# AndrewRLawrence/dp_gp_lvm

Hardware: AMD Instinct MI355X
Metric: ELBO evals/sec (N=2000,D=512,M=128,Q=10) (higher is better)
Workload: dtype f32 (psi-statistics: f16 hi/lo-split MFMA operands, fp32 accumulate) + f64 (Cholesky chain)

## Files before the change

### dp_gp_lvm_amd/csrc/psi2_pairs.hip

```cpp
#include <type_traits>
#include "internal.h"
#include "psi2_consts.h"
#include "psi2_chain_task.h"

typedef _Float16 pp_h8 __attribute__((ext_vector_type(8)));
typedef _Float16 pp_h2 __attribute__((ext_vector_type(2)));
typedef float pp_f16v __attribute__((ext_vector_type(16)));

#define PP_APAD 8
#define PP_LDS_HDR 512

#ifndef PP_G
#define PP_G(KS) ((KS) <= 4 ? 6 : ((KS) <= 6 ? 4 : 2))
#endif
#ifndef PP_WAVES
#define PP_WAVES 2
#endif
template <int KS> struct PairsCfg { static constexpr int G = PP_G(KS); };

#ifndef PP_NW8_MIN_TILES
#define PP_NW8_MIN_TILES 512
#endif
#ifndef PP_DEEP_PREFETCH
#define PP_DEEP_PREFETCH 1
#endif
#ifndef PP_SCALAR_ADD
#define PP_SCALAR_ADD 1
#endif

template <int KS, int GG, int NW>
__device__ __forceinline__ void pairs_load(pp_h8 (&bop)[GG][KS], int tb, const _Float16 *__restrict__ img, int l5, int half) {
#pragma unroll
    for (int g = 0; g < GG; ++g) {
        const pp_h8 *row = reinterpret_cast<const pp_h8 *>(img) + (size_t)(tb + NW * g) * KS * 64 + 32 * half + l5;
#pragma unroll
        for (int ks = 0; ks < KS; ++ks) bop[g][ks] = row[ks * 64];
    }
}

template <int KS, int GG, int NW>
__device__ __forceinline__ void pairs_group(int tb, pp_h8 (&bop)[GG][KS], int tb_next, const _Float16 *__restrict__ aimg,
                                            const _Float16 *__restrict__ img,
                                            const unsigned *__restrict__ pmap, const float *__restrict__ scale, int ntile,
                                            int l5, int half, float poison, float *__restrict__ out, int Mp, int chunk) {
    constexpr int SLP = 16 * KS, LDA = SLP + PP_APAD;
    static_assert(GG == 1 || (GG & 1) == 0, "ping-pong needs an even number of resident tiles");
    unsigned pm[GG];
    float sc[GG], old[GG];
#pragma unroll
    for (int g = 0; g < GG; ++g) {
        pm[g] = pmap[32 * (tb + NW * g) + l5];
        sc[g] = scale[32 * (tb + NW * g) + l5];
    }
#pragma unroll
    for (int g = 0; g < GG; ++g) {
        old[g] = 0.0f;
        if (chunk && pm[g] != 0xffffffffu && half == 0) old[g] = out[(size_t)(pm[g] >> 16) * Mp + (pm[g] & 0xffffu)];
    }
    float acc[GG][4];
#pragma unroll
    for (int g = 0; g < GG; ++g)
#pragma unroll
        for (int i = 0; i < 4; ++i) acc[g][i] = 0.0f;
    const _Float16 *arow = aimg + (size_t)l5 * LDA + 8 * half;
    auto load_a = [&](pp_h8 (&a)[KS], int nt) __attribute__((always_inline)) {
#ifdef PP_DIAG_NO_ALOAD
        if (nt > 1) return;
#endif
#pragma unroll
        for (int ks = 0; ks < KS; ++ks) a[ks] = *reinterpret_cast<const pp_h8 *>(arow + (size_t)nt * 32 * LDA + 16 * ks);
    };
    auto mma = [&](pp_f16v &c, const pp_h8 (&a)[KS], const pp_h8 (&bq)[KS]) __attribute__((always_inline)) {
#pragma unroll
        for (int v = 0; v < 16; ++v) c[v] = 0.0f;
#pragma unroll
        for (int ks = 0; ks < KS; ++ks) c = __builtin_amdgcn_mfma_f32_32x32x16_f16(a[ks], bq[ks], c, 0, 0, 0);
    };
    auto stage = [&](pp_f16v &cn, const pp_h8 (&a)[KS], const pp_h8 (&bq)[KS], float (&ac)[4], const pp_f16v &cu)
                     __attribute__((always_inline)) {
#pragma unroll
        for (int v = 0; v < 16; ++v) cn[v] = 0.0f;
#ifndef PP_MFMA_PER_STEP
#define PP_MFMA_PER_STEP 1
#endif
#pragma unroll
        for (int ks = 0; ks < KS; ks += PP_MFMA_PER_STEP) {
#ifndef PP_DIAG_NO_MFMA
#pragma unroll
            for (int k2 = ks; k2 < ks + PP_MFMA_PER_STEP && k2 < KS; ++k2)
                cn = __builtin_amdgcn_mfma_f32_32x32x16_f16(a[k2], bq[k2], cn, 0, 0, 0);
#endif
            __builtin_amdgcn_sched_barrier(0);
            const int kend = (ks + PP_MFMA_PER_STEP < KS) ? ks + PP_MFMA_PER_STEP : KS;
            const int v0 = (16 * ks) / KS, v1 = (16 * kend) / KS;
#pragma unroll
            for (int v = v0; v < v1; ++v) {
#ifdef PP_DIAG_NO_EXP
                const float e = cu[v];
#else
                const float e = __builtin_amdgcn_exp2f(cu[v]);
#endif
#if PP_SCALAR_ADD
                asm("v_add_f32 %0, %0, %1" : "+v"(ac[v & 3]) : "v"(e));
#else
                ac[v & 3] += e;
#endif
            }
            __builtin_amdgcn_sched_barrier(0);
        }
    };
    pp_f16v c0, c1;
    if constexpr (GG == 2 && PP_DEEP_PREFETCH) {
        pp_h8 a0[KS], a1[KS], a2[KS];
        load_a(a0, 0);
        load_a(a1, min(1, ntile - 1));
        mma(c0, a0, bop[0]);
#pragma unroll 1
        for (int nt = 0; nt < ntile; nt += 3) {
            load_a(a2, min(nt + 2, ntile - 1));
            stage(c1, a0, bop[1], acc[0], c0);
            stage(c0, a1, bop[0], acc[1], c1);
            if (nt + 1 >= ntile) break;
            load_a(a0, min(nt + 3, ntile - 1));
            stage(c1, a1, bop[1], acc[0], c0);
            stage(c0, a2, bop[0], acc[1], c1);
            if (nt + 2 >= ntile) break;
            load_a(a1, min(nt + 4, ntile - 1));
            stage(c1, a2, bop[1], acc[0], c0);
            stage(c0, a0, bop[0], acc[1], c1);
        }
    } else {
        pp_h8 a_0[KS], a_1[KS];
        load_a(a_0, 0);
        mma(c0, a_0, bop[0]);
        auto row = [&](const pp_h8 (&a_cur)[KS], const pp_h8 (&a_nxt)[KS]) __attribute__((always_inline)) {
            if constexpr (GG == 1) {
                stage(c1, a_nxt, bop[0], acc[0], c0);
                c0 = c1;
            } else {
#pragma unroll
                for (int g = 0; g < GG; g += 2) {
                    stage(c1, a_cur, bop[g + 1], acc[g], c0);
                    if (g + 2 < GG) stage(c0, a_cur, bop[g + 2], acc[g + 1], c1);
                    else stage(c0, a_nxt, bop[0], acc[g + 1], c1);
                }
            }
        };
#pragma unroll 1
        for (int nt = 0; nt < ntile; nt += 2) {
            load_a(a_1, min(nt + 1, ntile - 1));
            row(a_0, a_1);
            if (nt + 1 >= ntile) break;
            load_a(a_0, min(nt + 2, ntile - 1));
            row(a_1, a_0);
        }
    }
    if (tb_next >= 0) pairs_load<KS, GG, NW>(bop, tb_next, img, l5, half);
#pragma unroll
    for (int g = 0; g < GG; ++g) {
        float tot = (acc[g][0] + acc[g][1]) + (acc[g][2] + acc[g][3]);
        tot += __shfl_xor(tot, 32, 64);
        if (pm[g] != 0xffffffffu && half == 0)
            out[(size_t)(pm[g] >> 16) * Mp + (pm[g] & 0xffffu)] = old[g] + (sc[g] * tot + poison);
    }
}

template <typename TIN>
__global__ __launch_bounds__(256) void psi2_pair_scale_kernel(int M, int Q, const TIN *__restrict__ z,
                                                              const TIN *__restrict__ gamma, const TIN *__restrict__ alpha,
                                                              float *__restrict__ scale) {
    psi2_pair_scale_block<TIN, TIN>((int)blockIdx.y, (int)blockIdx.x, M, Q, z, gamma, alpha, scale);
}

template <typename TIN, int KS, int NW>
__global__ __launch_bounds__(64 * NW, PP_WAVES) void psi2_pairs_kernel(int N, int M, int Q, int B, const unsigned char *__restrict__ consts,
                                                            const TIN *__restrict__ mu, const TIN *__restrict__ s,
                                                            const TIN *__restrict__ gamma, const float *__restrict__ scale,
                                                            float *__restrict__ part, int Mp, int n_per_split, int n_splits,
                                                            int n_ranges, int tiles_per_range, int R, ChainKTask task) {
    constexpr int G = PairsCfg<KS>::G, SLP = 16 * KS, LDA = SLP + PP_APAD;
    extern __shared__ __align__(16) unsigned char smem_raw[];
    int item;
    if (psi2_task_1d(blockIdx.x, task.ws ? B : 0, task.last != 0, item)) {
#ifndef PP_NO_CHAIN
        if constexpr (std::is_same<TIN, double>::value && NW == 4) chain_k_task<2>(task, item, smem_raw);
#endif
        return;
    }
    const int b = item % B, sp = (item / B) % n_splits, rg = item / (B * n_splits);
    float *gq = reinterpret_cast<float *>(smem_raw);
    float *zc = gq + 32;
    _Float16 *aimg = reinterpret_cast<_Float16 *>(smem_raw + PP_LDS_HDR);
    const Psi2Consts C = psi2_consts_layout(M, Q);
    const _Float16 *img = reinterpret_cast<const _Float16 *>(consts + C.off_pairs);
    const unsigned *pmap = reinterpret_cast<const unsigned *>(consts + C.off_pmap);
    const float *sc_b = scale + (size_t)b * C.Ppad;
    const int t = threadIdx.x, lane = t & 63, l5 = lane & 31, half = lane >> 5;
    const int wv = __builtin_amdgcn_readfirstlane(t >> 6);
    if (t < 32) {
        gq[t] = (t < Q) ? (float)gamma[(size_t)b * Q + t] : 0.0f;
        zc[t] = reinterpret_cast<const float *>(consts)[t];
    }
    const int tiles_total = C.Ppad / 32;
    const int t0 = rg * tiles_per_range, t1 = min(tiles_total, t0 + tiles_per_range);
    const int nbeg = sp * n_per_split, nend = min(N, nbeg + n_per_split);
    float poison = 0.0f;
    float *out = part + ((size_t)sp * B + b) * (size_t)Mp * Mp;
    bool oor = false;
    __syncthreads();

    for (int n0 = nbeg, chunk = 0; n0 < nend; n0 += R, ++chunk) {
        const int rows = min(R, nend - n0), ntile = (rows + 31) >> 5;
        if (chunk) __syncthreads();
        for (int r = t; r < 32 * ntile; r += 64 * NW) {
            const int n = n0 + r;
            unsigned *dst = reinterpret_cast<unsigned *>(aimg + (size_t)r * LDA);
            float cc = -60000.0f;
            if (n < nend) {
                cc = 0.0f;
                for (int q = 0; q < Q; ++q) {
                    const float g = gq[q], sv = (float)s[(size_t)n * Q + q], mc = (float)mu[(size_t)n * Q + q] - zc[q];
                    const float den = 2.0f * g * sv + 1.0f, w = g / den;
                    const float a = dpgp_pin((float)(-0.25 * DPGP_LOG2E / PSI2_PAIR_S2_SCALE) * w);
                    const float bb = dpgp_pin((float)DPGP_LOG2E * w * mc);
                    cc -= bb * mc + 0.5f * __builtin_amdgcn_logf(den);
                    const _Float16 ah = (_Float16)a, alo = (_Float16)(a - (float)ah);
                    const _Float16 bh = (_Float16)bb, blo = (_Float16)(bb - (float)bh);
                    const pp_h2 w0 = {ah, ah}, w1 = {alo, bh}, w2 = {bh, blo};
                    dst[3 * q] = __builtin_bit_cast(unsigned, w0);
                    dst[3 * q + 1] = __builtin_bit_cast(unsigned, w1);
                    dst[3 * q + 2] = __builtin_bit_cast(unsigned, w2);
                }
                oor |= !(cc >= -8192.0f);
                cc = fmaxf(cc, -60000.0f);
            } else {
                for (int q = 0; q < 3 * Q; ++q) dst[q] = 0u;
            }
            cc = dpgp_pin(cc);
            const _Float16 ch = (_Float16)cc;
            const float r1 = dpgp_pin(cc - (float)ch);
            const _Float16 cm = (_Float16)r1;
            const pp_h2 cw = {ch, cm}, cw2 = {(_Float16)(r1 - (float)cm), (_Float16)0.0f};
            dst[3 * Q] = __builtin_bit_cast(unsigned, cw);
            for (int k = 3 * Q + 1; k < SLP / 2; ++k) dst[k] = 0u;
            if (6 * Q + 2 < SLP) dst[3 * Q + 1] = __builtin_bit_cast(unsigned, cw2);
        }
        if (__syncthreads_or(oor ? 1 : 0)) poison = __builtin_nanf("");

        int tb = t0 + wv;
        if (tb + NW * (G - 1) < t1) {
            pp_h8 bop[G][KS];
            pairs_load<KS, G, NW>(bop, tb, img, l5, half);
            for (; tb + NW * (G - 1) < t1; tb += NW * G) {
                const int nx = tb + NW * G;
                pairs_group<KS, G, NW>(tb, bop, nx + NW * (G - 1) < t1 ? nx : -1, aimg, img, pmap, sc_b, ntile, l5, half, poison, out,
                                   Mp, chunk);
            }
        }
        if constexpr (G > 2)
            for (; tb + NW < t1; tb += 2 * NW) {
                pp_h8 bop[2][KS];
                pairs_load<KS, 2, NW>(bop, tb, img, l5, half);
                pairs_group<KS, 2, NW>(tb, bop, -1, aimg, img, pmap, sc_b, ntile, l5, half, poison, out, Mp, chunk);
            }
        for (; tb < t1; tb += NW) {
            pp_h8 bop[1][KS];
            pairs_load<KS, 1, NW>(bop, tb, img, l5, half);
            pairs_group<KS, 1, NW>(tb, bop, -1, aimg, img, pmap, sc_b, ntile, l5, half, poison, out, Mp, chunk);
        }
    }
}

struct PairsGeom {
    int KS, R, n_ranges, tiles_per_range, NW;
    size_t lds;
};
static PairsGeom pairs_geom(int B, int N, int M, int Q, int ns, size_t chain_lds) {
    const Psi2Consts C = psi2_consts_layout(M, Q);
    PairsGeom g;
    g.KS = C.KS;
    const size_t row = sizeof(_Float16) * (size_t)(16 * C.KS + PP_APAD);
    size_t budget = 80 * 1024;
    if (const char *e = getenv("DPGP_PP_LDS_KB")) budget = (size_t)atoi(e) * 1024;
    if (chain_lds > budget) budget = chain_lds;
    int rmax = (int)((budget - PP_LDS_HDR) / row) & ~31;
    const int nper = dpgp_ceil_div(N, ns);
    g.NW = (!chain_lds && nper > rmax && C.Ppad / 32 >= PP_NW8_MIN_TILES) ? 8 : 4;
    if (const char *e = getenv("DPGP_PP_NW")) {
        const int v = atoi(e);
        if ((v == 4 || v == 8) && !(v == 8 && chain_lds)) g.NW = v;
    }
    if (g.NW == 8) {
        budget = 160 * 1024;
        rmax = (int)((budget - PP_LDS_HDR) / row) & ~31;
    }
    int r = dpgp_round_up(nper, 32);
    if (r > rmax) {
        const int chunks = dpgp_ceil_div(nper, rmax);
        r = dpgp_round_up(dpgp_ceil_div(nper, chunks), 32);
    }
    g.R = r;
    g.lds = PP_LDS_HDR + row * (size_t)r;
    if (chain_lds > g.lds) g.lds = chain_lds;
    const int tiles = C.Ppad / 32;
    int nr = chain_lds ? (B < 128 ? 512 - B : 512) / (B * ns) : dpgp_ceil_div(g.NW == 8 ? 256 : 512, B * ns);
    if (nr > dpgp_ceil_div(tiles, 32)) nr = dpgp_ceil_div(tiles, 32);
    if (nr < 1) nr = 1;
    if (const char *e = getenv("DPGP_PP_RANGES")) {
        const int v = atoi(e);
        if (v >= 1 && v <= tiles) nr = v;
    }
    g.tiles_per_range = dpgp_ceil_div(tiles, nr);
    g.n_ranges = dpgp_ceil_div(tiles, g.tiles_per_range);
    return g;
}

template <typename TIN, int KS, int NW>
static int launch_pairs_ks(int B, int N, int M, int Q, const TIN *mu, const TIN *s, const TIN *gamma, const float *scale,
                           float *part, int ns, const ChainKTask &task, const unsigned char *consts, const PairsGeom &g,
                           hipStream_t st) {
    const int Mp = dpgp_round_up(M, 16);
    const int nper = dpgp_ceil_div(N, ns);
    const long long nwg = (long long)B * ns * g.n_ranges + (task.ws ? B : 0);
    if (nwg > 0x7fffffffLL) return -1;
    auto kern = psi2_pairs_kernel<TIN, KS, NW>;
    if (NW == 8 && task.ws) return -16;
    if (g.lds > 48 * 1024 &&
        hipFuncSetAttribute(reinterpret_cast<const void *>(kern), hipFuncAttributeMaxDynamicSharedMemorySize, (int)g.lds) !=
            hipSuccess)
        return DPGP_ERR_LAUNCH;
    DPGP_PRELAUNCH(); hipLaunchKernelGGL(kern, dim3((unsigned)nwg), dim3(64 * NW), g.lds, st, N, M, Q, B, consts, mu, s, gamma, scale, part,
                       Mp, nper, ns, g.n_ranges, g.tiles_per_range, g.R, task);
    DPGP_LAUNCH_CHECK();
    return DPGP_OK;
}

size_t psi2_pairs_scale_bytes(int B, int M) {
    const size_t ppad = ((size_t)M * (M + 1) / 2 + 31) & ~(size_t)31;
    return dpgp_align256(sizeof(float) * (size_t)B * ppad);
}
template <typename TIN>
int launch_psi2_pairs(int B, int N, int M, int Q, const TIN *z, const TIN *mu, const TIN *s, const TIN *gamma,
                      const TIN *alpha, float *part, int ns, const ChainKTask &task, const unsigned char *consts, float *scale,
                      int scale_ready, hipStream_t st) {
    if (!consts || !scale) return -18;
    if (!scale_ready) {
        const Psi2Consts C = psi2_consts_layout(M, Q);
        DPGP_PRELAUNCH(); hipLaunchKernelGGL((psi2_pair_scale_kernel<TIN>), dim3(dpgp_ceil_div(C.Ppad, 256), B), dim3(256), 0, st, M, Q, z,
                           gamma, alpha, scale);
        DPGP_LAUNCH_CHECK();
    }
    size_t chain_lds = 0;
    if (task.ws) {
        if (!chain_k_resident(task.Mp, task.elem)) return -16;
        chain_lds = chain_k_lds_bytes(task.Mp, task.elem);
    }
    const PairsGeom g = pairs_geom(B, N, M, Q, ns, chain_lds);
    switch (g.KS) {
#define CASE(k)                                                                                                       \
    case k:                                                                                                           \
        return g.NW == 8 ? launch_pairs_ks<TIN, k, 8>(B, N, M, Q, mu, s, gamma, scale, part, ns, task, consts, g, st) \
                         : launch_pairs_ks<TIN, k, 4>(B, N, M, Q, mu, s, gamma, scale, part, ns, task, consts, g, st);
        CASE(2) CASE(4) CASE(6) CASE(8)
#undef CASE
    }
    return -4;
}
template int launch_psi2_pairs<float>(int, int, int, int, const float *, const float *, const float *, const float *,
                                      const float *, float *, int, const ChainKTask &, const unsigned char *, float *, int,
                                      hipStream_t);
template int launch_psi2_pairs<double>(int, int, int, int, const double *, const double *, const double *, const double *,
                                       const double *, float *, int, const ChainKTask &, const unsigned char *, float *, int,
                                       hipStream_t);
```

Measured before the change: 771.5.

## Peel final pipeline iteration and overlap next-group B-operand refill with tail MFMAs

Restructures the psi2 pairs MFMA pipeline so the last row is peeled out of the loop. The B-operand registers for the next tile group are refilled one slot at a time, interleaved with the tail stage and drain, instead of being loaded all at once after the loop. This is meant to hide the global-load latency of the next group behind the remaining MFMA/exp work and to avoid the redundant clamped tail iteration. It adds a REFILL template parameter and changes loop bounds, which risks edge-case bugs for small ntile values and adds register pressure.

```diff
diff --git a/dp_gp_lvm_amd/csrc/psi2_pairs.hip b/dp_gp_lvm_amd/csrc/psi2_pairs.hip
--- a/dp_gp_lvm_amd/csrc/psi2_pairs.hip
+++ b/dp_gp_lvm_amd/csrc/psi2_pairs.hip
@@ -28,6 +28,19 @@
 #define PP_SCALAR_ADD 1
 #endif
 
+__device__ __forceinline__ void pairs_accumulate(float &acc, float x) {
+#ifdef PP_DIAG_NO_EXP
+    const float e = x;
+#else
+    const float e = __builtin_amdgcn_exp2f(x);
+#endif
+#if PP_SCALAR_ADD
+    acc = dpgp_pin(acc + e);
+#else
+    acc += e;
+#endif
+}
+
 template <int KS, int GG, int NW>
 __device__ __forceinline__ void pairs_load(pp_h8 (&bop)[GG][KS], int tb, const _Float16 *__restrict__ img, int l5, int half) {
 #pragma unroll
@@ -38,7 +51,7 @@
     }
 }
 
-template <int KS, int GG, int NW>
+template <int KS, int GG, int NW, bool REFILL>
 __device__ __forceinline__ void pairs_group(int tb, pp_h8 (&bop)[GG][KS], int tb_next, const _Float16 *__restrict__ aimg,
                                             const _Float16 *__restrict__ img,
                                             const unsigned *__restrict__ pmap, const float *__restrict__ scale, int ntile,
@@ -94,20 +107,26 @@
             const int kend = (ks + PP_MFMA_PER_STEP < KS) ? ks + PP_MFMA_PER_STEP : KS;
             const int v0 = (16 * ks) / KS, v1 = (16 * kend) / KS;
 #pragma unroll
-            for (int v = v0; v < v1; ++v) {
-#ifdef PP_DIAG_NO_EXP
-                const float e = cu[v];
-#else
-                const float e = __builtin_amdgcn_exp2f(cu[v]);
-#endif
-#if PP_SCALAR_ADD
-                asm("v_add_f32 %0, %0, %1" : "+v"(ac[v & 3]) : "v"(e));
-#else
-                ac[v & 3] += e;
-#endif
-            }
+            for (int v = v0; v < v1; ++v) pairs_accumulate(ac[v & 3], cu[v]);
             __builtin_amdgcn_sched_barrier(0);
         }
+    };
+    auto drain = [&](float (&ac)[4], const pp_f16v &cu) __attribute__((always_inline)) {
+#pragma unroll
+        for (int v = 0; v < 16; ++v) pairs_accumulate(ac[v & 3], cu[v]);
+        __builtin_amdgcn_sched_barrier(0);
+    };
+    auto refill = [&](int g) __attribute__((always_inline)) {
+        if constexpr (!REFILL) return;
+        const pp_h8 *src = reinterpret_cast<const pp_h8 *>(img) + (size_t)(tb_next + NW * g) * KS * 64;
+        const unsigned lo = 32u * half + l5;
+#pragma unroll
+        for (int ks = 0; ks < KS; ++ks) bop[g][ks] = src[ks * 64 + lo];
+        __builtin_amdgcn_sched_barrier(0);
+    };
+    auto copy_a = [&](pp_h8 (&d)[KS], const pp_h8 (&a)[KS]) __attribute__((always_inline)) {
+#pragma unroll
+        for (int ks = 0; ks < KS; ++ks) d[ks] = a[ks];
     };
     pp_f16v c0, c1;
     if constexpr (GG == 2 && PP_DEEP_PREFETCH) {
@@ -116,19 +135,23 @@
         load_a(a1, min(1, ntile - 1));
         mma(c0, a0, bop[0]);
 #pragma unroll 1
-        for (int nt = 0; nt < ntile; nt += 3) {
+        for (int nt = 0; nt + 1 < ntile; nt += 3) {
             load_a(a2, min(nt + 2, ntile - 1));
             stage(c1, a0, bop[1], acc[0], c0);
             stage(c0, a1, bop[0], acc[1], c1);
-            if (nt + 1 >= ntile) break;
+            if (nt + 2 >= ntile) { copy_a(a0, a1); break; }
             load_a(a0, min(nt + 3, ntile - 1));
             stage(c1, a1, bop[1], acc[0], c0);
             stage(c0, a2, bop[0], acc[1], c1);
-            if (nt + 2 >= ntile) break;
+            if (nt + 3 >= ntile) { copy_a(a0, a2); break; }
             load_a(a1, min(nt + 4, ntile - 1));
             stage(c1, a2, bop[1], acc[0], c0);
             stage(c0, a0, bop[0], acc[1], c1);
         }
+        refill(0);
+        stage(c1, a0, bop[1], acc[0], c0);
+        refill(1);
+        drain(acc[1], c1);
     } else {
         pp_h8 a_0[KS], a_1[KS];
         load_a(a_0, 0);
@@ -147,15 +170,31 @@
             }
         };
 #pragma unroll 1
-        for (int nt = 0; nt < ntile; nt += 2) {
-            load_a(a_1, min(nt + 1, ntile - 1));
+        for (int nt = 0; nt + 1 < ntile; nt += 2) {
+            load_a(a_1, nt + 1);
             row(a_0, a_1);
-            if (nt + 1 >= ntile) break;
-            load_a(a_0, min(nt + 2, ntile - 1));
+            if (nt + 2 >= ntile) break;
+            load_a(a_0, nt + 2);
             row(a_1, a_0);
         }
-    }
-    if (tb_next >= 0) pairs_load<KS, GG, NW>(bop, tb_next, img, l5, half);
+        load_a(a_0, ntile - 1);
+        refill(0);
+        if constexpr (GG == 1) {
+            drain(acc[0], c0);
+        } else {
+#pragma unroll
+            for (int g = 0; g < GG; g += 2) {
+                stage(c1, a_0, bop[g + 1], acc[g], c0);
+                refill(g + 1);
+                if (g + 2 < GG) {
+                    stage(c0, a_0, bop[g + 2], acc[g + 1], c1);
+                    refill(g + 2);
+                } else {
+                    drain(acc[g + 1], c1);
+                }
+            }
+        }
+    }
 #pragma unroll
     for (int g = 0; g < GG; ++g) {
         float tot = (acc[g][0] + acc[g][1]) + (acc[g][2] + acc[g][3]);
@@ -251,22 +290,21 @@
         if (tb + NW * (G - 1) < t1) {
             pp_h8 bop[G][KS];
             pairs_load<KS, G, NW>(bop, tb, img, l5, half);
-            for (; tb + NW * (G - 1) < t1; tb += NW * G) {
-                const int nx = tb + NW * G;
-                pairs_group<KS, G, NW>(tb, bop, nx + NW * (G - 1) < t1 ? nx : -1, aimg, img, pmap, sc_b, ntile, l5, half, poison, out,
-                                   Mp, chunk);
-            }
+            for (; tb + NW * (2 * G - 1) < t1; tb += NW * G)
+                pairs_group<KS, G, NW, true>(tb, bop, tb + NW * G, aimg, img, pmap, sc_b, ntile, l5, half, poison, out, Mp, chunk);
+            pairs_group<KS, G, NW, false>(tb, bop, -1, aimg, img, pmap, sc_b, ntile, l5, half, poison, out, Mp, chunk);
+            tb += NW * G;
         }
         if constexpr (G > 2)
             for (; tb + NW < t1; tb += 2 * NW) {
                 pp_h8 bop[2][KS];
                 pairs_load<KS, 2, NW>(bop, tb, img, l5, half);
-                pairs_group<KS, 2, NW>(tb, bop, -1, aimg, img, pmap, sc_b, ntile, l5, half, poison, out, Mp, chunk);
+                pairs_group<KS, 2, NW, false>(tb, bop, -1, aimg, img, pmap, sc_b, ntile, l5, half, poison, out, Mp, chunk);
             }
         for (; tb < t1; tb += NW) {
             pp_h8 bop[1][KS];
             pairs_load<KS, 1, NW>(bop, tb, img, l5, half);
-            pairs_group<KS, 1, NW>(tb, bop, -1, aimg, img, pmap, sc_b, ntile, l5, half, poison, out, Mp, chunk);
+            pairs_group<KS, 1, NW, false>(tb, bop, -1, aimg, img, pmap, sc_b, ntile, l5, half, poison, out, Mp, chunk);
         }
     }
 }
```

Measured after the change: 788.3 (median of 6 runs). 2.2% higher.
